# lucastrefezza/quadruplet-sentence-transformer

Measured on AMD Instinct MI355X. Metric: quadruplets/sec (seq_len=128, all-MiniLM-L6-v2) training step, higher is better.
Workload: dtype bf16; 1 GPU; all-MiniLM-L6-v2 dims (random-init), 64 quadruplets/GPU x 1 GPU, seq_len=128, fwd + gamma-quadruplet loss + bwd + clip + AdamW, dropout 0.1 on hidden states and attention probabilities as the reference's train() mode (BASELINE.json configs[1]); global_batch=64, seq_len=128, parallelism=dp1, precision=bf16 MFMA operands, fp32 accumulate/residual/LN/softmax/loss/optimizer, launch=eager

## Files before the change

### include/qst_kernels.h

```cpp
#pragma once
#include <stddef.h>
#include <stdint.h>

#ifdef __cplusplus
extern "C" {
#endif

enum {
    QST_EPI_BF16 = 0,
    QST_EPI_F32_RESID = 1,
    QST_EPI_GELU = 2,
    QST_EPI_GELU_BWD = 3,
    QST_EPI_F32_RESID_BF16 = 4,
    QST_EPI_GELU_MX = 5,
    QST_EPI_GELU_MX_TRAIN = 6
};

typedef struct {
    const uint32_t* state;
    uint32_t site;
    uint32_t thr16;
} QstDrop;
#define QST_DROP_SITE_EMBED 0xE0u
#define QST_DROP_SITE_ATTN_OUT(layer) (4u * (uint32_t)(layer) + 0u)
// ... 19 lines not shown
    void* C3;
    void* C4;
    const void* B2;
    int32_t b2_n0;
    int32_t sat16;
} QstGemmArgs;

int qst_gemm_nt(const QstGemmArgs* a, int epi, void* stream);
int qst_gemm_nt_f8(const QstGemmArgs* a, int epi, void* stream);
int qst_quant_mx(const void* src, int src_is_bf16, int64_t rows, int K, void* q, void* scales, void* stream);
typedef struct {
    const float* gamma;
    const float* beta;
    float eps;
    void* xhat;
    float* rstd;
    float* partials;
} QstLnEpi;
int qst_gemm_nt_ln_supported(int N);
int qst_gemm_nt_ln_block_rows(int N);
int qst_gemm_nt_ln_block_rows_m(int N, int M);
int qst_gemm_nt_ln(const QstGemmArgs* a, const QstLnEpi* ln, int mode, void* stream);
int qst_gemm_nt8_ln_supported(int N);
int qst_gemm_nt8_ln_block_rows(int M, int N);
int qst_gemm_nt8_ln(const QstGemmArgs* a, const QstLnEpi* ln, int mode, void* stream);
int qst_gemm_nt8_ln_timeouts(void);
int qst_gemm_nt8_f8_ln(const QstGemmArgs* a, const QstLnEpi* ln, void* stream);
typedef struct {
    const void* A;
    const void* B1;
    const void* B2;
    const float* bias1;
    const float* bias2;
    const float* resid;
    const void* aux;
    void* save_gp;
    void* save_h;
    float* C;
    void* C2;
    int32_t M, H, I;
    int32_t diag;
} QstFfnArgs;
int qst_ffn_chain_supported(int H, int I);
int qst_ffn_chain(const QstFfnArgs* a, const QstLnEpi* ln, int mode, void* stream);
int qst_gemm_tn(const QstGemmArgs* a, void* stream);
#define QST_TN_MAX_PROB 8
typedef struct {
    int32_t nprob;
    int32_t splits;
    int32_t total_tiles;
    int32_t ranges_per_xcd;
    int32_t tiles[QST_TN_MAX_PROB];
    QstGemmArgs prob[QST_TN_MAX_PROB];
} QstTnGroup;
int qst_gemm_tn_group(const QstTnGroup* grp, void* stream);

int qst_gemm8_stagger(int cycles);
int qst_gemm8_ln_store(int mode);
int qst_gemm_nt8_supported(const QstGemmArgs* a, int epi);
int qst_gemm_nt8(const QstGemmArgs* a, int epi, int tile, void* stream);
int qst_gemm_tn8_group(const QstTnGroup* grp, void* stream);
int qst_gemm_nt8_f8(const QstGemmArgs* a, int epi, int tile, void* stream);
int qst_gemm8_mode(int mode);

int qst_embed_ln_fwd(const int64_t* ids, const int64_t* type_ids, const int32_t* pos_ids,
                     const float* word_emb, const float* pos_emb, const float* type_emb,
                     const float* gamma, const float* beta, float eps, int M, int H,
                     float* y, void* y_bf16, void* xhat_bf16, float* rstd, void* stream);
int qst_embed_ln_fwd_drop(const int64_t* ids, const int64_t* type_ids, const int32_t* pos_ids,
                          const float* word_emb, const float* pos_emb, const float* type_emb,
                          const float* gamma, const float* beta, float eps, int M, int H,
                          float* y, void* y_bf16, void* xhat_bf16, float* rstd, const QstDrop* drop, void* stream);
int qst_ln_fwd(const float* s, const float* gamma, const float* beta, float eps, int M, int H,
               float* y, void* y_bf16, void* xhat_bf16, float* rstd, void* stream);
int qst_ln_fwd_mx(const float* s, const float* gamma, const float* beta, float eps, int M, int H,
                  float* y, void* y_bf16, void* yq, void* ys, void* stream);
int qst_embed_ln_fwd_mx(const int64_t* ids, const int64_t* type_ids, const int32_t* pos_ids,
                        const float* word_emb, const float* pos_emb, const float* type_emb,
                        const float* gamma, const float* beta, float eps, int M, int H,
                        float* y, void* y_bf16, void* yq, void* ys, void* stream);
int qst_ln_fwd_mx_train(const float* s, const float* gamma, const float* beta, float eps, int M, int H, float* y,
                        void* y_bf16, void* xhat_bf16, float* rstd, void* yq, void* ys, void* stream);
int qst_embed_ln_fwd_mx_train(const int64_t* ids, const int64_t* type_ids, const int32_t* pos_ids,
                              const float* word_emb, const float* pos_emb, const float* type_emb,
                              const float* gamma, const float* beta, float eps, int M, int H, float* y,
                              void* y_bf16, void* xhat_bf16, float* rstd, void* yq, void* ys,
                              const QstDrop* drop , void* stream);
size_t qst_ln_bwd_scratch_bytes(int M, int H);
int qst_ln_bwd(const float* dy, const void* xhat_bf16, const float* rstd, const float* gamma, int M, int H,
               float* ds, void* ds_bf16, float* dgamma, float* dbeta, float* scratch, void* stream);
int qst_ln_bwd_drop(const float* dy, const void* xhat_bf16, const float* rstd, const float* gamma, int M, int H,
                    float* ds, void* ds_bf16, float* dgamma, float* dbeta, float* scratch,
                    const QstDrop* drop_in, const QstDrop* drop_out, void* stream);
#define QST_LN_BATCH_MAX 32
typedef struct {
    int32_t count, H, nblocks;
    const float* partials[QST_LN_BATCH_MAX];
    float* dgamma[QST_LN_BATCH_MAX];
    float* dbeta[QST_LN_BATCH_MAX];
    int32_t nblocks_each[QST_LN_BATCH_MAX];
} QstLnReduceBatch;
int qst_ln_bwd_reduce_batch(const QstLnReduceBatch* b, void* stream);
int qst_embed_bwd(const float* ds, const int64_t* ids, const int64_t* type_ids, const int32_t* pos_ids,
                  int nseq, int L, int H, int num_types, float* dword, float* dpos, float* dtype_, void* stream);
int qst_position_ids(const int64_t* ids, int nseq, int L, int arch, int pad_id, int32_t* pos_ids, void* stream);
int qst_forward_prologue(const int64_t* ids, int nseq, int L, int arch, int pad_id, int32_t* pos_ids,
                         uint32_t* drop_state, uint32_t* drop_snapshot, void* stream);

// ... 121 lines not shown
```

### quadruplet-sentence-transformer_amd/_lib.py

```python
from __future__ import annotations

import ctypes as C
import os
from typing import Optional

_HERE = os.path.dirname(os.path.abspath(__file__))
LIB_PATH = os.path.join(_HERE, "libqst.so")

c_i64p = C.POINTER(C.c_int64)
c_i32p = C.POINTER(C.c_int32)
c_f32p = C.POINTER(C.c_float)
vp = C.c_void_p


class QstError(RuntimeError):
    pass


class QstConfig(C.Structure):
    _fields_ = [("arch", C.c_int32), ("vocab_size", C.c_int32), ("hidden_size", C.c_int32),
                ("num_layers", C.c_int32), ("num_heads", C.c_int32), ("intermediate_size", C.c_int32),
                ("max_position", C.c_int32), ("type_vocab_size", C.c_int32), ("layer_norm_eps", C.c_float),
                ("normalize", C.c_int32), ("rel_buckets", C.c_int32), ("rel_max_distance", C.c_int32),
                ("pad_token_id", C.c_int32), ("precision", C.c_int32)]


class QstDrop(C.Structure):
    _fields_ = [("state", vp), ("site", C.c_uint32), ("thr16", C.c_uint32)]


class QstAttnDesc(C.Structure):
    _fields_ = [("qkv", vp), ("mask", vp), ("rel_pos", vp), ("nseq", C.c_int32), ("L", C.c_int32), ("A", C.c_int32),
                ("d", C.c_int32), ("ctx", vp), ("lse", vp), ("dctx", vp), ("dqkv", vp), ("drel", vp), ("delta_scratch", vp),
                ("force_split", C.c_int32), ("drop", QstDrop)]


class QstGemmArgs(C.Structure):
    _fields_ = [("A", vp), ("B", vp), ("C", vp), ("C2", vp), ("aux", vp), ("bias", vp), ("resid", vp),
                ("colsum", vp), ("M", C.c_int32), ("N", C.c_int32), ("K", C.c_int32), ("lda", C.c_int32),
                ("ldb", C.c_int32), ("ldc", C.c_int32), ("ldr", C.c_int32), ("splits", C.c_int32), ("bscale", vp),
                ("drop", QstDrop), ("drop_where", C.c_int32), ("C3", vp), ("C4", vp), ("B2", vp), ("b2_n0", C.c_int32), ("sat16", C.c_int32)]


class QstLnEpi(C.Structure):
    _fields_ = [("gamma", vp), ("beta", vp), ("eps", C.c_float), ("xhat", vp), ("rstd", vp), ("partials", vp)]


class QstFfnArgs(C.Structure):
    _fields_ = [("A", vp), ("B1", vp), ("B2", vp), ("bias1", vp), ("bias2", vp), ("resid", vp), ("aux", vp),
                ("save_gp", vp), ("save_h", vp), ("C", vp), ("C2", vp), ("M", C.c_int32), ("H", C.c_int32), ("I", C.c_int32),
                ("diag", C.c_int32)]


class QstLnReduceBatch(C.Structure):
    _fields_ = [("count", C.c_int32), ("H", C.c_int32), ("nblocks", C.c_int32), ("partials", vp * 32), ("dgamma", vp * 32),
                ("dbeta", vp * 32), ("nblocks_each", C.c_int32 * 32)]


class QstTnGroup(C.Structure):
    _fields_ = [("nprob", C.c_int32), ("splits", C.c_int32), ("total_tiles", C.c_int32), ("ranges_per_xcd", C.c_int32),
                ("tiles", C.c_int32 * 8),
                ("prob", QstGemmArgs * 8)]


SIGNATURES = {
    "qst_strerror": (C.c_char_p, [C.c_int]),
    "qst_last_hip_error": (C.c_int, []),
    "qst_version": (C.c_int, []),
    "qst_arena_elems": (C.c_int64, [C.POINTER(QstConfig)]),
    "qst_arena_num_segments": (C.c_int, [C.POINTER(QstConfig)]),
    "qst_arena_segment": (C.c_int, [C.POINTER(QstConfig), C.c_int, C.POINTER(C.c_char_p), c_i64p, c_i64p, c_i32p, c_i32p]),
    "qst_shadow_elems": (C.c_int64, [C.POINTER(QstConfig)]),
    "qst_encoder_create": (C.c_int, [C.POINTER(QstConfig), C.POINTER(vp)]),
    "qst_encoder_destroy": (None, [vp]),
    "qst_encoder_saved_bytes": (C.c_size_t, [vp, C.c_int, C.c_int, C.c_int]),
    "qst_encoder_bwd_workspace_bytes": (C.c_size_t, [vp, C.c_int, C.c_int]),
    "qst_refresh_shadow": (C.c_int, [vp, vp, vp, vp]),
    "qst_refresh_shadow_mx": (C.c_int, [vp, vp, vp, vp]),
    "qst_encoder_forward": (C.c_int, [vp, vp, vp, vp, C.c_int, C.c_int, vp, vp, vp, vp, vp, C.c_size_t, C.c_int, vp]),
    "qst_encoder_backward": (C.c_int, [vp, vp, vp, vp, C.c_int, C.c_int, vp, vp, vp, vp, vp, C.c_size_t, vp, C.c_size_t, vp]),
    "qst_encoder_backward_partial": (C.c_int, [vp, vp, vp, vp, C.c_int, C.c_int, vp, vp, vp, vp, vp, C.c_size_t, vp, C.c_size_t,
                                               C.c_int, C.c_int, C.c_int, C.c_int, vp]),
    "qst_encoder_backward_stage": (C.c_int, [vp, vp, vp, vp, C.c_int, C.c_int, vp, vp, vp, vp, vp, C.c_size_t, vp, C.c_size_t,
                                             C.c_int, C.c_int, C.c_int, vp]),
    "qst_quadruplet_loss": (C.c_int, [vp, vp, vp, vp, C.c_int, C.c_int, C.c_float, C.c_float, C.c_float, C.c_float,
                                      C.c_float, C.c_int, C.c_int, vp, vp, vp, vp, vp, vp, vp, vp]),
    "qst_pair_metric": (C.c_int, [vp, vp, C.c_int, C.c_int, C.c_int, vp, vp, vp, vp, vp]),
    "qst_pair_loss": (C.c_int, [vp, vp, vp, C.c_int, C.c_int, C.c_int, C.c_int, C.c_float, C.c_int, vp, vp, vp, vp, vp, vp]),
    "qst_triplet_loss": (C.c_int, [vp, vp, vp, C.c_int, C.c_int, C.c_int, C.c_float, C.c_int, vp, vp, vp, vp, vp, vp, vp]),
    "qst_quadruplet_eval": (C.c_int, [vp, vp, vp, vp, C.c_int, C.c_int, vp, vp, vp, vp]),
    "qst_mnrl_workspace_bytes": (C.c_size_t, [C.c_int, C.c_int, C.c_int]),
    "qst_mnrl_loss": (C.c_int, [vp, vp, C.c_int, C.c_int, C.c_int, C.c_int, C.c_float, C.c_int, vp, vp, vp, vp, vp, C.c_size_t,
                                vp]),
    "qst_batch_triplet_workspace_bytes": (C.c_size_t, [C.c_int, C.c_int]),
    "qst_batch_triplet_loss": (C.c_int, [vp, vp, C.c_int, C.c_int, C.c_int, C.c_int, C.c_float, vp, vp, vp, vp, vp, C.c_size_t,
                                         vp]),
    "qst_embed_mse": (C.c_int, [vp, vp, C.c_int, C.c_int, vp, vp, vp, vp, vp]),
    "qst_margin_mse_loss": (C.c_int, [vp, vp, vp, vp, C.c_int, C.c_int, C.c_int, C.c_int, vp, vp, vp, vp, vp, vp, vp, vp]),
    "qst_clip_adamw_step": (C.c_int, [vp, vp, vp, vp, vp, C.c_float, C.c_float, C.c_float, C.c_float, C.c_float,
                                      C.c_float, C.c_float, C.c_int64, vp, vp, vp]),
    "qst_shadow8_bytes": (C.c_int64, [C.POINTER(QstConfig)]),
    "qst_clip_adamw_step_sched": (C.c_int, [vp, vp, vp, vp, vp, C.c_float, C.c_float, C.c_float, C.c_float, C.c_float,
                                            C.c_float, C.c_float, C.c_int64, C.c_int64, vp, vp, vp, vp]),
    "qst_topk_workspace_bytes": (C.c_size_t, [C.c_int, C.c_int, C.c_int]),
    "qst_topk_scores": (C.c_int, [vp, vp, C.c_int, C.c_int, C.c_int, C.c_int, C.c_int, vp, vp, vp, C.c_size_t, vp]),
    "qst_topk_scores_capped": (C.c_int, [vp, vp, C.c_int, C.c_int, C.c_int, C.c_int, C.c_int, C.c_float, vp, vp, vp,
                                         C.c_size_t, vp]),
    "qst_score_workspace_bytes": (C.c_size_t, [C.c_int, C.c_int, C.c_int]),
    "qst_score_matrix": (C.c_int, [vp, vp, C.c_int, C.c_int, C.c_int, C.c_int, vp, C.c_int64, vp, C.c_size_t, vp]),
    "qst_gemm_nt": (C.c_int, [C.POINTER(QstGemmArgs), C.c_int, vp]),
    "qst_gemm_nt_f8": (C.c_int, [C.POINTER(QstGemmArgs), C.c_int, vp]),
    "qst_quant_mx": (C.c_int, [vp, C.c_int, C.c_int64, C.c_int, vp, vp, vp]),
    "qst_gemm_nt_ln_supported": (C.c_int, [C.c_int]),
    "qst_gemm_nt_ln": (C.c_int, [C.POINTER(QstGemmArgs), C.POINTER(QstLnEpi), C.c_int, vp]),
    "qst_gemm_nt_ln_block_rows": (C.c_int, [C.c_int]),
    "qst_gemm_nt_ln_block_rows_m": (C.c_int, [C.c_int, C.c_int]),
    "qst_gemm_nt8_ln_block_rows": (C.c_int, [C.c_int, C.c_int]),
    "qst_gemm8_stagger": (C.c_int, [C.c_int]),
    "qst_gemm8_ln_store": (C.c_int, [C.c_int]),
    "qst_gemm_nt8_ln_supported": (C.c_int, [C.c_int]),
    "qst_gemm_nt8_ln": (C.c_int, [C.POINTER(QstGemmArgs), C.POINTER(QstLnEpi), C.c_int, vp]),
    "qst_gemm_nt8_ln_timeouts": (C.c_int, []),
    "qst_gemm_nt8_f8_ln": (C.c_int, [C.POINTER(QstGemmArgs), C.POINTER(QstLnEpi), vp]),
    "qst_ffn_chain_supported": (C.c_int, [C.c_int, C.c_int]),
    "qst_ffn_chain": (C.c_int, [C.POINTER(QstFfnArgs), C.POINTER(QstLnEpi), C.c_int, vp]),
    "qst_gemm_tn": (C.c_int, [C.POINTER(QstGemmArgs), vp]),
    "qst_gemm_tn_group": (C.c_int, [C.POINTER(QstTnGroup), vp]),
    "qst_gemm_nt8_supported": (C.c_int, [C.POINTER(QstGemmArgs), C.c_int]),
    "qst_gemm_nt8": (C.c_int, [C.POINTER(QstGemmArgs), C.c_int, C.c_int, vp]),
    "qst_gemm_tn8_group": (C.c_int, [C.POINTER(QstTnGroup), vp]),
    "qst_gemm_nt8_f8": (C.c_int, [C.POINTER(QstGemmArgs), C.c_int, C.c_int, vp]),
    "qst_gemm8_mode": (C.c_int, [C.c_int]),
    "qst_embed_ln_fwd": (C.c_int, [vp, vp, vp, vp, vp, vp, vp, vp, C.c_float, C.c_int, C.c_int, vp, vp, vp, vp, vp]),
    "qst_embed_ln_fwd_drop": (C.c_int, [vp, vp, vp, vp, vp, vp, vp, vp, C.c_float, C.c_int, C.c_int, vp, vp, vp, vp,
                                        C.POINTER(QstDrop), vp]),
    "qst_ln_fwd_mx": (C.c_int, [vp, vp, vp, C.c_float, C.c_int, C.c_int, vp, vp, vp, vp, vp]),
    "qst_embed_ln_fwd_mx": (C.c_int, [vp, vp, vp, vp, vp, vp, vp, vp, C.c_float, C.c_int, C.c_int, vp, vp, vp, vp, vp]),
    "qst_ln_fwd_mx_train": (C.c_int, [vp, vp, vp, C.c_float, C.c_int, C.c_int, vp, vp, vp, vp, vp, vp, vp]),
    "qst_embed_ln_fwd_mx_train": (C.c_int, [vp, vp, vp, vp, vp, vp, vp, vp, C.c_float, C.c_int, C.c_int, vp, vp, vp, vp, vp, vp,
                                            vp, vp]),
    "qst_ln_fwd": (C.c_int, [vp, vp, vp, C.c_float, C.c_int, C.c_int, vp, vp, vp, vp, vp]),
    "qst_ln_bwd_scratch_bytes": (C.c_size_t, [C.c_int, C.c_int]),
    "qst_ln_bwd_reduce_batch": (C.c_int, [vp, vp]),
    "qst_ln_bwd": (C.c_int, [vp, vp, vp, vp, C.c_int, C.c_int, vp, vp, vp, vp, vp, vp]),
    "qst_ln_bwd_drop": (C.c_int, [vp, vp, vp, vp, C.c_int, C.c_int, vp, vp, vp, vp, vp, C.POINTER(QstDrop), C.POINTER(QstDrop), vp]),
    "qst_embed_bwd": (C.c_int, [vp, vp, vp, vp, C.c_int, C.c_int, C.c_int, C.c_int, vp, vp, vp, vp]),
    "qst_position_ids": (C.c_int, [vp, C.c_int, C.c_int, C.c_int, C.c_int, vp, vp]),
    "qst_forward_prologue": (C.c_int, [vp, C.c_int, C.c_int, C.c_int, C.c_int, vp, vp, vp, vp]),
    "qst_pool_norm_fwd": (C.c_int, [vp, vp, C.c_int, C.c_int, C.c_int, C.c_int, vp, vp, vp]),
    "qst_pool_norm_bwd": (C.c_int, [vp, vp, vp, C.c_int, C.c_int, C.c_int, C.c_int, vp, vp]),
    "qst_pool_fwd": (C.c_int, [vp, vp, C.c_int, C.c_int, C.c_int, C.c_int, C.c_int, vp, vp, vp, vp]),
    "qst_pool_bwd": (C.c_int, [vp, vp, vp, vp, C.c_int, C.c_int, C.c_int, C.c_int, C.c_int, vp, vp]),
    "qst_attention_fwd": (C.c_int, [vp, vp, vp, C.c_int, C.c_int, C.c_int, C.c_int, vp, vp, vp]),
    "qst_attention_bwd": (C.c_int, [vp, vp, vp, vp, vp, vp, C.c_int, C.c_int, C.c_int, C.c_int, vp, vp, vp, vp]),
    "qst_attention_fwd_ex": (C.c_int, [C.POINTER(QstAttnDesc), vp]),
    "qst_attention_bwd_ex": (C.c_int, [C.POINTER(QstAttnDesc), vp]),
    "qst_dropout_multipliers": (C.c_int, [C.POINTER(QstDrop), C.c_int, C.c_int64, vp, vp]),
    "qst_abi_sizeof": (C.c_int64, [C.c_int]),
    "qst_normalize_rows": (C.c_int, [vp, C.c_int, C.c_int, vp, vp]),
    "qst_cls_head_fwd": (C.c_int, [vp, C.c_int64, C.c_int, C.c_int, vp, vp, vp, vp, C.c_int, C.c_int, C.c_int, vp, vp]),
    "qst_dropout_init": (C.c_int, [vp, C.c_uint64, vp]),
    "qst_dropout_advance": (C.c_int, [vp, vp]),
    "qst_encoder_set_dropout": (C.c_int, [vp, C.c_float, C.c_float, vp]),
    "qst_encoder_set_ffn_chain": (C.c_int, [vp, C.c_int]),
    "qst_encoder_set_ln_fusion": (C.c_int, [vp, C.c_int]),
    "qst_encoder_set_pooling": (C.c_int, [vp, C.c_int]),
    "qst_encoder_embedding_dim": (C.c_int, [vp]),
    "qst_transpose_f32": (C.c_int, [vp, C.c_int, C.c_int, C.c_int, vp, C.c_int, vp]),
    "qst_gelu_f32": (C.c_int, [vp, C.c_int64, vp, vp]),
    "qst_gelu_bwd_f32": (C.c_int, [vp, vp, C.c_int64, vp, vp]),
    "qst_colsum_f32": (C.c_int, [vp, C.c_int, C.c_int, C.c_int, vp, vp]),
    "qst_embed_sum_f32": (C.c_int, [vp, vp, vp, vp, vp, vp, C.c_int, C.c_int, vp, vp]),
    "qst_ln_bwd_f32": (C.c_int, [vp, vp, vp, C.c_float, C.c_int, C.c_int, vp, vp, vp, vp]),
    "qst_attention_bwd_f32": (C.c_int, [vp, vp, vp, vp, vp, C.c_int, C.c_int, C.c_int, C.c_int, vp, vp, vp]),
    "qst_attention_bwd_f32_drop": (C.c_int, [vp, vp, vp, vp, vp, C.c_int, C.c_int, C.c_int, C.c_int, vp, vp, vp, vp]),
    "qst_attention_bwd_x3_scratch_bytes": (C.c_size_t, [C.c_int, C.c_int, C.c_int]),
    "qst_attention_bwd_x3": (C.c_int, [vp, vp, vp, vp, vp, C.c_int, C.c_int, C.c_int, C.c_int, vp, vp, vp, vp, vp]),
    "qst_dropout_apply_f32": (C.c_int, [vp, vp, vp, C.c_int64, vp, vp]),
    "qst_comm_unique_id": (C.c_int, [vp]),
    "qst_comm_init": (C.c_int, [C.c_int, C.c_int, vp, C.POINTER(vp)]),
# ... 82 lines not shown
```

### quadruplet-sentence-transformer_amd/csrc/gemm.hip

```cpp
#include "qst_common.h"
#include "qst_kernels.h"

namespace {

constexpr uint32_t kOOB = 0x7FFFFFF0u;

typedef __attribute__((address_space(3))) void lds_void;
typedef __attribute__((ext_vector_type(2))) float f32x2;

template <bool ONCE = false>
__device__ __forceinline__ void dma16(__amdgpu_buffer_rsrc_t r, char* lds_wave_base, uint32_t voff, uint32_t soff) {
    __builtin_amdgcn_raw_ptr_buffer_load_lds(r, (lds_void*)lds_wave_base, 16, (int)voff, (int)soff, 0,
                                             (ONCE && QST_STREAM_LOADS) ? 2 : 0);
}
template <int N> __device__ __forceinline__ void wait_vmcnt() {
    if (N == 0) asm volatile("s_waitcnt vmcnt(0)" ::: "memory");
    else if (N == 4) asm volatile("s_waitcnt vmcnt(4)" ::: "memory");
    else asm volatile("s_waitcnt vmcnt(8)" ::: "memory");
}
template <int N> __device__ __forceinline__ void wait_vmcnt_n() {
    if (N == 0) asm volatile("s_waitcnt vmcnt(0)" ::: "memory");
    else if (N == 6) asm volatile("s_waitcnt vmcnt(6)" ::: "memory");
    else if (N == 12) asm volatile("s_waitcnt vmcnt(12)" ::: "memory");
    else if (N == 18) asm volatile("s_waitcnt vmcnt(18)" ::: "memory");
    else asm volatile("s_waitcnt vmcnt(24)" ::: "memory");
}
__device__ __forceinline__ void wait_stage(int stages_behind) {
    if (stages_behind >= 2) wait_vmcnt<8>();
    else if (stages_behind == 1) wait_vmcnt<4>();
    else wait_vmcnt<0>();
}

__device__ __forceinline__ int xcd_remap(int b, int nwg) {
    const int q = nwg >> 3, r = nwg & 7, x = b & 7;
    return (x < r ? x * (q + 1) : r * (q + 1) + (x - r) * q) + (b >> 3);
}

constexpr int NBK = 64;
constexpr int NT_STG_LD = 100;
__device__ __forceinline__ uint32_t nt_off(int row, int chunk) {
    return (uint32_t)(row * 128 + ((chunk ^ ((row >> 1) & 7)) << 4));
}

struct NoHook { __device__ __forceinline__ void operator()() const {} };
template <int WAVES_M, int WAVES_N, typename HOOK = NoHook, bool A_ONCE = false, int A_SLOTS = 2, bool SPLITW = true>
__device__ __forceinline__ void nt_mainloop(const QstGemmArgs& g, char* smem, int m0, int n0, f32x16 (&acc)[2][3],
                                            HOOK after_first_issue = HOOK()) {
    constexpr int NBM = 64 * WAVES_M, NBN = 96 * WAVES_N, NW = WAVES_M * WAVES_N;
    constexpr int NT_A_BYTES = NBM * NBK * 2, NT_B_BYTES = NBN * NBK * 2;
    constexpr int NT_STAGE = NT_A_BYTES + NT_B_BYTES;
    constexpr int A_PER_WAVE = (NBM / 8) / NW;
    constexpr int B_PER_WAVE = (NBN / 8) / NW;
// ... 724 lines not shown
                    s2 += v[t][0] * x[t][0] + v[t][1] * x[t][1];
                }
                const float m1 = wave_sum(s1) * inv_n, m2 = wave_sum(s2) * inv_n;
                if (m < g.M) {
#pragma unroll
                    for (int t = 0; t < 3; ++t) {
                        const int c = 2 * (lane + 64 * t);
                        f32x2 o;
                        o[0] = rs[i][k] * (v[t][0] - m1 - x[t][0] * m2);
                        o[1] = rs[i][k] * (v[t][1] - m1 - x[t][1] * m2);
                        st_stream((f32x2*)((float*)g.C + (size_t)m * g.ldc + c), o);
                        if (g.C2) {
                            if (DROP && dwhere == 2) {
                                float k0, k1;
                                drop_pair(dc, (uint32_t)m * LN_N + c, k0, k1);
                                o[0] *= k0; o[1] *= k1;
                            }
                            st_stream((uint32_t*)((op16*)g.C2 + (size_t)m * g.ldc + c), pack_op2(o[0], o[1]));
                        }
                    }
                }
            }
        }
        LN_STAMP(4 + 2 * i);
    }
    LN_STAMP(7);
    if (MODE == 1 && e.partials) {
        __syncthreads();
        float* red = (float*)smem;
#pragma unroll
        for (int t = 0; t < 3; ++t) {
            *(f32x2*)(red + (wave * 2 + 0) * LN_N + 2 * (lane + 64 * t)) = ag[t];
            *(f32x2*)(red + (wave * 2 + 1) * LN_N + 2 * (lane + 64 * t)) = ab[t];
        }
        __syncthreads();
        for (int c = tid; c < 2 * LN_N; c += 512) {
            const int which = c / LN_N, n = c - which * LN_N;
            float a = 0.f;
#pragma unroll
            for (int w = 0; w < 8; ++w) a += red[(w * 2 + which) * LN_N + n];
            e.partials[(size_t)blockIdx.x * 2 * LN_N + c] = a;
        }
    }
}

constexpr int TT = 192, TBK = 64, TSTAGES = 3;
constexpr int TT_TILE = TBK * TT * 2;
constexpr int TT_STAGE = 2 * TT_TILE;
constexpr int TT_LDS = TSTAGES * TT_STAGE;
__device__ __forceinline__ int tn_swz(int row) { return ((row >> 1) & 1) << 2; }
__device__ __forceinline__ uint32_t tn_off(int row, int chunk) {
    return (uint32_t)(row * 384 + ((chunk ^ tn_swz(row)) << 4));
}
__device__ __forceinline__ op16x4 lds_tr16(const char* p) {
    return lds_tr16_op(p);
}
__device__ __forceinline__ op16x4 lds_tr16_at(uint32_t a) {
    typedef __attribute__((ext_vector_type(4))) __bf16 raw4;
    return __builtin_bit_cast(op16x4, __builtin_amdgcn_ds_read_tr16_b64_v4bf16((__attribute__((address_space(3))) raw4*)(uintptr_t)a));
}

__global__ __launch_bounds__(512, 1) void gemm_tn_group_kernel(QstTnGroup grp) {
    extern __shared__ __attribute__((aligned(16))) char smem[];
    const int tid = threadIdx.x, lane = tid & 63;
    const int wave = __builtin_amdgcn_readfirstlane(tid >> 6);
    const int wm = (wave >> 1) & 1, wn = wave & 1;
    const int xcd = blockIdx.x & 7, jloc = blockIdx.x >> 3;
    const int wg_per_range = (int)(gridDim.x >> 3) / grp.ranges_per_xcd;
    const int range = xcd + 8 * (jloc / wg_per_range);
    const int jr = jloc % wg_per_range;
    const int M = grp.prob[0].M;
    const int per = (((M + grp.splits - 1) / grp.splits) + TBK - 1) / TBK * TBK;
    const int mbeg = range * per, mend = min(M, mbeg + per);
    if (mbeg >= mend) return;
    const int S = (mend - mbeg + TBK - 1) / TBK;
    const int W = wg_per_range, T = grp.total_tiles;
    const int a_full = T / W, b_left = T % W;
    const int pieces = b_left > 0 ? max(1, W / b_left) : 1;
    const int ntasks = a_full + ((b_left > 0 && jr / pieces < b_left) ? 1 : 0);

    const int li = lane & 15, q = li >> 2, p = li & 3, gsel = (lane >> 4) & 1, fh = lane >> 5;
    const int fr = lane & 31;

#pragma unroll 1
    for (int task = 0; task < ntasks; ++task) {
        int tile, s0, s1;
        if (task < a_full) { tile = task * W + jr; s0 = 0; s1 = S; }
        else {
            tile = a_full * W + jr / pieces;
            const int pc = jr % pieces;
            const int per_piece = (S + pieces - 1) / pieces;
            s0 = pc * per_piece; s1 = min(S, s0 + per_piece);
        }
        const int nm = s1 - s0;
        if (nm <= 0) continue;
        int pi = 0;
#pragma unroll 1
        while (pi + 1 < grp.nprob && tile >= grp.tiles[pi]) { tile -= grp.tiles[pi]; ++pi; }
        const QstGemmArgs& g = grp.prob[pi];
        const int ntk = (g.K + TT - 1) / TT;
        const int n0 = (tile / ntk) * TT, k0 = (tile % ntk) * TT;
        const int row0 = mbeg + s0 * TBK;

        if (wave >= 4) {
            const bool isA = wave < 6;
            const int half = wave & 1;
            const int ld = isA ? g.lda : g.ldb, c0 = isA ? n0 : k0, width = isA ? g.N : g.K;
            const op16* base = (const op16*)(isA ? g.A : g.B) + (size_t)row0 * ld + c0;
            const uint32_t bytes = (uint32_t)min((size_t)(mend - row0) * ld * 2u - (size_t)c0 * 2u, (size_t)0x7FFFFF00u);
            const __amdgpu_buffer_rsrc_t rs = make_rsrc(base, bytes);
            constexpr int NDMA = TBK * 24 / 64 / 2;
            uint32_t vo[NDMA];
#pragma unroll
            for (int b = 0; b < 3; ++b) {
                const int pp = (half * NDMA + b) * 64 + lane;
                const int row = pp / 24, chunk = (pp % 24) ^ tn_swz(row);
                const bool ok = c0 + chunk * 8 < width;
#pragma unroll
                for (int t = b; t < NDMA; t += 3)
                    vo[t] = ok ? (uint32_t)(row + 8 * (t / 3)) * ld * 2u + chunk * 16u : kOOB;
            }
            auto issue = [&](int mt) {
                char* st = smem + (mt % TSTAGES) * TT_STAGE + (isA ? 0 : TT_TILE);
                const uint32_t so = (uint32_t)mt * TBK * ld * 2u;
#pragma unroll
                for (int t = 0; t < NDMA; ++t) dma16(rs, st + (half * NDMA + t) * 1024, vo[t], so);
            };
            constexpr int AHEAD = TSTAGES - 1;
#pragma unroll 1
            for (int st = 0; st < AHEAD && st < nm; ++st) issue(st);
#pragma unroll 1
            for (int mt = 0; mt < nm; ++mt) {
                const int younger = min(AHEAD - 1, nm - 1 - mt);
                if (younger >= 1) wait_vmcnt_n<12>(); else wait_vmcnt_n<0>();
                __builtin_amdgcn_s_barrier();
                if (mt + AHEAD < nm) issue(mt + AHEAD);
            }
            __builtin_amdgcn_s_barrier();
            continue;
        }

        f32x16 acc[3][3];
        float bsum[3] = {0.f, 0.f, 0.f};
#pragma unroll
        for (int i = 0; i < 3; ++i)
#pragma unroll
            for (int j = 0; j < 3; ++j)
#pragma unroll
                for (int r = 0; r < 16; ++r) acc[i][j][r] = 0.f;
        const bool do_bias = (g.colsum != nullptr) && (k0 == 0) && (wn == 0);
        uint32_t la[3], lb[3];
        {
            const uint32_t lr = (uint32_t)(8 * fh + q) * 384u + 8u * (p & 1), g2 = gsel * 2 + (p >> 1);
#pragma unroll
            for (int i = 0; i < 3; ++i) {
                la[i] = lr + (uint32_t)(((wm * 12 + i * 4 + g2) ^ tn_swz(q)) << 4);
                lb[i] = lr + TT_TILE + (uint32_t)(((wn * 12 + i * 4 + g2) ^ tn_swz(q)) << 4);
            }
        }
        uint32_t slot = (uint32_t)(uintptr_t)(__attribute__((address_space(3))) char*)smem;

        for (int mt = 0; mt < nm; ++mt) {
            __builtin_amdgcn_s_barrier();
            uint32_t ra[3], rb[3];
#pragma unroll
            for (int i = 0; i < 3; ++i) {
                ra[i] = slot + la[i]; rb[i] = slot + lb[i];
                asm volatile("" : "+v"(ra[i]), "+v"(rb[i]));
            }
            slot = (mt % TSTAGES == TSTAGES - 1) ? slot - (TSTAGES - 1) * TT_STAGE : slot + TT_STAGE;
            op16x8 fa[2][3], fb[2][3];
#define TN_LOAD(ks_, set_)                                                                                  \
    do {                                                                                                    \
        _Pragma("unroll") for (int i = 0; i < 3; ++i) {                                                     \
            _Pragma("unroll") for (int jj = 0; jj < 2; ++jj) {                                              \
                const op16x4 ta = lds_tr16_at(ra[i] + ((ks_) * 16 + 4 * jj) * 384);                         \
                const op16x4 tb = lds_tr16_at(rb[i] + ((ks_) * 16 + 4 * jj) * 384);                         \
                _Pragma("unroll") for (int e = 0; e < 4; ++e) { fa[set_][i][jj * 4 + e] = ta[e]; fb[set_][i][jj * 4 + e] = tb[e]; } \
            }                                                                                               \
        }                                                                                                   \
    } while (0)
#define TN_MFMA(set_)                                                                                       \
    do {                                                                                                    \
        _Pragma("unroll") for (int i = 0; i < 3; ++i)                                                       \
            _Pragma("unroll") for (int j = 0; j < 3; ++j)                                                   \
                acc[i][j] = mfma32_op(fa[set_][i], fb[set_][j], acc[i][j]); \
        if (do_bias) {    \
            _Pragma("unroll") for (int i = 0; i < 3; ++i)                                                   \
                _Pragma("unroll") for (int e = 0; e < 8; ++e) bsum[i] += (float)fa[set_][i][e];             \
        }                                                                                                   \
    } while (0)
            TN_LOAD(0, 0);
            TN_LOAD(1, 1);
            TN_MFMA(0);
            TN_LOAD(2, 0);
            TN_MFMA(1);
            TN_LOAD(3, 1);
            TN_MFMA(0);
            TN_MFMA(1);
#undef TN_LOAD
#undef TN_MFMA
            if (!do_bias) {
                __builtin_amdgcn_sched_group_barrier(0x100, 12, 0);
#pragma unroll
                for (int rep = 0; rep < 3; ++rep) {
#pragma unroll
                    for (int u = 0; u < 3; ++u) {
                        __builtin_amdgcn_sched_group_barrier(0x008, 1, 0);
                        __builtin_amdgcn_sched_group_barrier(0x100, 2, 0);
                    }
#pragma unroll
                    for (int u = 0; u < 6; ++u) {
                        __builtin_amdgcn_sched_group_barrier(0x008, 1, 0);
                        __builtin_amdgcn_sched_group_barrier(0x100, 1, 0);
                    }
                }
                __builtin_amdgcn_sched_group_barrier(0x008, 9, 0);
            }
        }
        __builtin_amdgcn_s_barrier();

        float* C = (float*)g.C;
#pragma unroll
        for (int j = 0; j < 3; ++j) {
            const int k = k0 + wn * 96 + j * 32 + fr;
            if (k >= g.K) continue;
#pragma unroll
            for (int i = 0; i < 3; ++i) {
#pragma unroll
                for (int r = 0; r < 16; ++r) {
                    const int n = n0 + wm * 96 + i * 32 + (r & 3) + 8 * (r >> 2) + 4 * fh;
                    if (n < g.N) atomicAdd(&C[(size_t)n * g.ldc + k], acc[i][j][r]);
                }
            }
        }
        if (do_bias) {
#pragma unroll
            for (int i = 0; i < 3; ++i) {
                const float t = bsum[i] + swap32(bsum[i]);
                const int n = n0 + wm * 96 + i * 32 + fr;
                if (fh == 0 && n < g.N) atomicAdd(&g.colsum[n], t);
            }
        }
    }
}

}

int qst_gemm8_mode_get();
static bool nt8_auto(const QstGemmArgs* a, int epi) {
    const int64_t tiles = (int64_t)((a->M + 255) / 256) * ((a->N + 255) / 256);
    if (tiles < 1024 || a->K < 768) return false;
    if (epi == QST_EPI_BF16) return true;
    if (epi == QST_EPI_GELU) return a->N >= 2304;
    if (epi == QST_EPI_GELU_BWD) return a->N >= 2304 && tiles >= 4096;
    if (epi == QST_EPI_F32_RESID || epi == QST_EPI_F32_RESID_BF16) return a->K >= 2304;
    return false;
}

template <int EPI, int WAVES_M, int WAVES_N = 2, int TI = 2>
static int launch_nt(const QstGemmArgs* a, hipStream_t st) {
    constexpr int NBM = 32 * TI * WAVES_M, NBN = 96 * WAVES_N;
    constexpr int lds = 2 * (NBM + NBN) * (TI == 4 ? 32 : NBK) * 2;
    static QstLdsAttr attr;
    if (int rc = qst_ensure_lds(attr, (const void*)gemm_nt_kernel<EPI, WAVES_M, WAVES_N, TI>, lds)) return rc;
    const int ntm = (a->M + NBM - 1) / NBM, ntn = (a->N + NBN - 1) / NBN;
    gemm_nt_kernel<EPI, WAVES_M, WAVES_N, TI><<<dim3(ntm * ntn), dim3(64 * WAVES_M * WAVES_N), lds, st>>>(*a);
    QST_LAUNCH_CHECK();
    return QST_OK;
}

extern "C" int QST_K(qst_gemm_nt)(const QstGemmArgs* a, int epi, void* stream) {
// ... 88 lines not shown
}

extern "C" int qst_quant_mx(const void* src, int src_is_bf16, int64_t rows, int K, void* q, void* scales, void* stream) {
    if (!src || !q || !scales || rows <= 0 || K <= 0) return QST_ERR_BAD_ARG;
    if (K % 32 != 0) return QST_ERR_UNSUPPORTED;
    const int64_t n8 = rows * K / 8;
    const unsigned grid = (unsigned)((n8 + 255) / 256);
    if (src_is_bf16) quant_mx_kernel<op16><<<grid, 256, 0, (hipStream_t)stream>>>((const op16*)src, n8, rows, K, (uint8_t*)q, (uint8_t*)scales);
    else quant_mx_kernel<float><<<grid, 256, 0, (hipStream_t)stream>>>((const float*)src, n8, rows, K, (uint8_t*)q, (uint8_t*)scales);
    QST_LAUNCH_CHECK();
    return QST_OK;
}

extern "C" int qst_gemm_nt_ln_supported(int N) { return (N == LN_N || qst_gemm_nt8_ln_supported(N)) ? 1 : 0; }
extern "C" int qst_gemm_nt_ln_block_rows(int N) { return N == LN_N ? 128 : 256; }
extern "C" int qst_gemm_nt_ln_block_rows_m(int N, int M) { return N == LN_N ? 128 : qst_gemm_nt8_ln_block_rows(M, N); }
#endif

extern "C" int QST_K(qst_gemm_nt_ln)(const QstGemmArgs* a, const QstLnEpi* ln, int mode, void* stream) {
    if (!a || !ln || !a->A || !a->B || !a->C || !ln->gamma || a->M <= 0 || a->K <= 0) return QST_ERR_BAD_ARG;
    if (mode != 0 && mode != 1) return QST_ERR_BAD_ARG;
    if (mode == 0 && !ln->beta) return QST_ERR_BAD_ARG;
    if (mode == 1 && (!ln->xhat || !ln->rstd)) return QST_ERR_BAD_ARG;
    if (a->N != LN_N && qst_gemm_nt8_ln_supported(a->N)) return QST_K(qst_gemm_nt8_ln)(a, ln, mode, stream);
    if (a->N != LN_N || a->K % NBK != 0 || a->lda % 8 != 0 || a->ldb % 8 != 0 || a->ldc % 2 != 0 || (a->resid && a->ldr % 2 != 0))
        return QST_ERR_UNSUPPORTED;
    if ((int64_t)128 * a->lda * 2 >= 0x7FFFFF00LL || (int64_t)LN_N * a->ldb * 2 >= 0x7FFFFF00LL) return QST_ERR_UNSUPPORTED;
    if (a->drop.thr16 && a->drop.state) {
        if (a->drop.thr16 > 65535u || (int64_t)a->M * a->N >= ((int64_t)1 << 32)) return QST_ERR_UNSUPPORTED;
        if (mode == 0 ? a->drop_where != 1 : (a->drop_where != 2 && a->drop_where != 3)) return QST_ERR_BAD_ARG;
    }
    static QstLdsAttr attr0, attr1, attr01, attr12, attr13;
    const int ntm = (a->M + 127) / 128;
    if (a->drop.thr16 && a->drop.state) {
        if (int rc = qst_ensure_lds(attr01, (const void*)gemm_nt_ln_kernel<0, 1>, LN_LDS)) return rc;
        if (int rc = qst_ensure_lds(attr12, (const void*)gemm_nt_ln_kernel<1, 2>, LN_LDS)) return rc;
        if (int rc = qst_ensure_lds(attr13, (const void*)gemm_nt_ln_kernel<1, 3>, LN_LDS)) return rc;
        if (mode == 0) gemm_nt_ln_kernel<0, 1><<<dim3(ntm), dim3(512), LN_LDS, (hipStream_t)stream>>>(*a, *ln);
        else if (a->drop_where == 2) gemm_nt_ln_kernel<1, 2><<<dim3(ntm), dim3(512), LN_LDS, (hipStream_t)stream>>>(*a, *ln);
        else gemm_nt_ln_kernel<1, 3><<<dim3(ntm), dim3(512), LN_LDS, (hipStream_t)stream>>>(*a, *ln);
        QST_LAUNCH_CHECK();
        return QST_OK;
    }
    if (int rc = qst_ensure_lds(attr0, (const void*)gemm_nt_ln_kernel<0>, LN_LDS)) return rc;
    if (int rc = qst_ensure_lds(attr1, (const void*)gemm_nt_ln_kernel<1>, LN_LDS)) return rc;
    if (mode == 0) gemm_nt_ln_kernel<0><<<dim3(ntm), dim3(512), LN_LDS, (hipStream_t)stream>>>(*a, *ln);
    else gemm_nt_ln_kernel<1><<<dim3(ntm), dim3(512), LN_LDS, (hipStream_t)stream>>>(*a, *ln);
    QST_LAUNCH_CHECK();
    return QST_OK;
}

static bool tn8_auto(const QstTnGroup* g) { (void)g; return false; }

extern "C" int QST_K(qst_gemm_tn_group)(const QstTnGroup* grp_in, void* stream) {
    if (!grp_in || grp_in->nprob <= 0 || grp_in->nprob > QST_TN_MAX_PROB) return QST_ERR_BAD_ARG;
    {
        const int mode = qst_gemm8_mode_get();
        if (mode >= 0 ? (mode & 2) != 0 : tn8_auto(grp_in)) return QST_K(qst_gemm_tn8_group)(grp_in, stream);
    }
    QstTnGroup g = *grp_in;
    g.total_tiles = 0;
    for (int i = 0; i < g.nprob; ++i) {
        const QstGemmArgs& a = g.prob[i];
        if (!a.A || !a.B || !a.C || a.M <= 0 || a.N <= 0 || a.K <= 0 || a.M != g.prob[0].M) return QST_ERR_BAD_ARG;
        if (a.lda % 8 != 0 || a.ldb % 8 != 0 || a.N % 8 != 0 || a.K % 8 != 0) return QST_ERR_UNSUPPORTED;
        if ((int64_t)a.M * a.lda * 2 >= 0x7FFFFF00LL || (int64_t)a.M * a.ldb * 2 >= 0x7FFFFF00LL) return QST_ERR_UNSUPPORTED;
        g.tiles[i] = ((a.N + TT - 1) / TT) * ((a.K + TT - 1) / TT);
        g.total_tiles += g.tiles[i];
    }
    const int M = g.prob[0].M;
    if (g.splits <= 0) {
        g.splits = 8;
    }
    g.splits = (g.splits + 7) / 8 * 8;
    g.ranges_per_xcd = g.splits / 8;
    const int64_t stages = ((int64_t)(M + g.splits - 1) / g.splits + TBK - 1) / TBK;
    int64_t wg_per_range = 32 / g.ranges_per_xcd;
    if (wg_per_range < 1) wg_per_range = 1;
    const int64_t work = (int64_t)g.total_tiles * stages;
    if (wg_per_range > work) wg_per_range = work < 1 ? 1 : work;
    const int grid = (int)(8 * g.ranges_per_xcd * wg_per_range);
    static QstLdsAttr attr;
    if (int rc = qst_ensure_lds(attr, (const void*)gemm_tn_group_kernel, TT_LDS)) return rc;
    gemm_tn_group_kernel<<<dim3(grid), dim3(512), TT_LDS, (hipStream_t)stream>>>(g);
    QST_LAUNCH_CHECK();
    return QST_OK;
}

extern "C" int QST_K(qst_gemm_tn)(const QstGemmArgs* a, void* stream) {
    if (!a) return QST_ERR_BAD_ARG;
    QstTnGroup g{};
    g.nprob = 1;
    g.splits = a->splits;
    g.prob[0] = *a;
    return QST_K(qst_gemm_tn_group)(&g, stream);
}
```

Before: 14330 quadruplets/s.

## Skew split-K row ranges and reorder leftover tiles in grouped TN GEMM

Replaces the uniform per-range row split in the weight-gradient TN GEMM with a skewed stage partition, so per-XCD ranges get unequal row counts. It also adds a by-piece ordering for leftover tiles, where odd pieces run their leftover task first, to balance workgroup finish times. The bias column-sum is now split across both wn halves by k-step parity and uses bf16 dot2 instead of scalar adds, which lets the MFMA schedule barriers stay on for bias tiles. The added template specialisation raises code size, and the skew changes how the atomic-add contention is distributed.

```diff
diff --git a/include/qst_kernels.h b/include/qst_kernels.h
--- a/include/qst_kernels.h
+++ b/include/qst_kernels.h
@@ -95,8 +95,11 @@
     int32_t ranges_per_xcd;
     int32_t tiles[QST_TN_MAX_PROB];
     QstGemmArgs prob[QST_TN_MAX_PROB];
+    int32_t skew;
+    int32_t order;
 } QstTnGroup;
 int qst_gemm_tn_group(const QstTnGroup* grp, void* stream);
+int qst_tn_group_ranges(const QstTnGroup* grp, int32_t* row_begin);
 
 int qst_gemm8_stagger(int cycles);
 int qst_gemm8_ln_store(int mode);
diff --git a/quadruplet-sentence-transformer_amd/_lib.py b/quadruplet-sentence-transformer_amd/_lib.py
--- a/quadruplet-sentence-transformer_amd/_lib.py
+++ b/quadruplet-sentence-transformer_amd/_lib.py
@@ -60,7 +60,8 @@
 class QstTnGroup(C.Structure):
     _fields_ = [("nprob", C.c_int32), ("splits", C.c_int32), ("total_tiles", C.c_int32), ("ranges_per_xcd", C.c_int32),
                 ("tiles", C.c_int32 * 8),
-                ("prob", QstGemmArgs * 8)]
+                ("prob", QstGemmArgs * 8),
+                ("skew", C.c_int32), ("order", C.c_int32)]
 
 
 SIGNATURES = {
@@ -126,6 +127,7 @@
     "qst_ffn_chain": (C.c_int, [C.POINTER(QstFfnArgs), C.POINTER(QstLnEpi), C.c_int, vp]),
     "qst_gemm_tn": (C.c_int, [C.POINTER(QstGemmArgs), vp]),
     "qst_gemm_tn_group": (C.c_int, [C.POINTER(QstTnGroup), vp]),
+    "qst_tn_group_ranges": (C.c_int, [C.POINTER(QstTnGroup), c_i32p]),
     "qst_gemm_nt8_supported": (C.c_int, [C.POINTER(QstGemmArgs), C.c_int]),
     "qst_gemm_nt8": (C.c_int, [C.POINTER(QstGemmArgs), C.c_int, C.c_int, vp]),
     "qst_gemm_tn8_group": (C.c_int, [C.POINTER(QstTnGroup), vp]),
diff --git a/quadruplet-sentence-transformer_amd/csrc/gemm.hip b/quadruplet-sentence-transformer_amd/csrc/gemm.hip
--- a/quadruplet-sentence-transformer_amd/csrc/gemm.hip
+++ b/quadruplet-sentence-transformer_amd/csrc/gemm.hip
@@ -1,3 +1,4 @@
+#include <type_traits>
 #include "qst_common.h"
 #include "qst_kernels.h"
 
@@ -828,12 +829,34 @@
 __device__ __forceinline__ uint32_t tn_off(int row, int chunk) {
     return (uint32_t)(row * 384 + ((chunk ^ tn_swz(row)) << 4));
 }
+__device__ __forceinline__ float add_pair(op16 a, op16 b, float c) {
+    const op16x2 v = {a, b}, one = {(op16)1.0f, (op16)1.0f};
+#if QST_OP_F16
+    return __builtin_amdgcn_fdot2(v, one, c, false);
+#else
+    return __builtin_amdgcn_fdot2_f32_bf16(v, one, c, false);
+#endif
+}
 __device__ __forceinline__ op16x4 lds_tr16(const char* p) {
     return lds_tr16_op(p);
 }
 __device__ __forceinline__ op16x4 lds_tr16_at(uint32_t a) {
     typedef __attribute__((ext_vector_type(4))) __bf16 raw4;
     return __builtin_bit_cast(op16x4, __builtin_amdgcn_ds_read_tr16_b64_v4bf16((__attribute__((address_space(3))) raw4*)(uintptr_t)a));
+}
+
+__host__ __device__ inline int tn_range_stage(int stages, int splits, int skew, int r) {
+    const int base = stages / splits, extra = stages % splits;
+    int s = r * base + (r > splits - extra ? r - (splits - extra) : 0);
+    if (skew > 0 && splits == 8) {
+        const int m = r < 8 - r ? r : 8 - r;
+        s -= skew * (m * (9 - m) / 2);
+    }
+    return s;
+}
+__host__ __device__ inline int tn_skew_max(int stages, int splits) {
+    const int base = stages / splits;
+    return splits == 8 && base > 1 ? (base - 1) / 4 : 0;
 }
 
 __global__ __launch_bounds__(512, 1) void gemm_tn_group_kernel(QstTnGroup grp) {
@@ -846,14 +869,19 @@
     const int range = xcd + 8 * (jloc / wg_per_range);
     const int jr = jloc % wg_per_range;
     const int M = grp.prob[0].M;
-    const int per = (((M + grp.splits - 1) / grp.splits) + TBK - 1) / TBK * TBK;
-    const int mbeg = range * per, mend = min(M, mbeg + per);
+    const int stages_m = (M + TBK - 1) / TBK;
+    const int mbeg = min(M, TBK * tn_range_stage(stages_m, grp.splits, grp.skew, range));
+    const int mend = min(M, TBK * tn_range_stage(stages_m, grp.splits, grp.skew, range + 1));
     if (mbeg >= mend) return;
     const int S = (mend - mbeg + TBK - 1) / TBK;
     const int W = wg_per_range, T = grp.total_tiles;
     const int a_full = T / W, b_left = T % W;
     const int pieces = b_left > 0 ? max(1, W / b_left) : 1;
-    const int ntasks = a_full + ((b_left > 0 && jr / pieces < b_left) ? 1 : 0);
+    const bool by_piece = grp.order == 2 && b_left > 0;
+    const int lt = by_piece ? jr % b_left : jr / pieces, lp = by_piece ? jr / b_left : jr % pieces;
+    const bool has_left = b_left > 0 && (by_piece ? lp < pieces : lt < b_left);
+    const bool left_first = by_piece && has_left && (lp & 1);
+    const int ntasks = a_full + (has_left ? 1 : 0);
 
     const int li = lane & 15, q = li >> 2, p = li & 3, gsel = (lane >> 4) & 1, fh = lane >> 5;
     const int fr = lane & 31;
@@ -861,12 +889,12 @@
 #pragma unroll 1
     for (int task = 0; task < ntasks; ++task) {
         int tile, s0, s1;
-        if (task < a_full) { tile = task * W + jr; s0 = 0; s1 = S; }
+        const int wt = left_first ? (task == 0 ? a_full : task - 1) : task;
+        if (wt < a_full) { tile = wt * W + jr; s0 = 0; s1 = S; }
         else {
-            tile = a_full * W + jr / pieces;
-            const int pc = jr % pieces;
+            tile = a_full * W + lt;
             const int per_piece = (S + pieces - 1) / pieces;
-            s0 = pc * per_piece; s1 = min(S, s0 + per_piece);
+            s0 = lp * per_piece; s1 = min(S, s0 + per_piece);
         }
         const int nm = s1 - s0;
         if (nm <= 0) continue;
@@ -924,7 +952,7 @@
             for (int j = 0; j < 3; ++j)
 #pragma unroll
                 for (int r = 0; r < 16; ++r) acc[i][j][r] = 0.f;
-        const bool do_bias = (g.colsum != nullptr) && (k0 == 0) && (wn == 0);
+        const bool do_bias = (g.colsum != nullptr) && (k0 == 0);
         uint32_t la[3], lb[3];
         {
             const uint32_t lr = (uint32_t)(8 * fh + q) * 384u + 8u * (p & 1), g2 = gsel * 2 + (p >> 1);
@@ -936,6 +964,8 @@
         }
         uint32_t slot = (uint32_t)(uintptr_t)(__attribute__((address_space(3))) char*)smem;
 
+        auto run_stages = [&](auto bias_tag) __attribute__((always_inline)) {
+        constexpr int BIAS = decltype(bias_tag)::value;
         for (int mt = 0; mt < nm; ++mt) {
             __builtin_amdgcn_s_barrier();
             uint32_t ra[3], rb[3];
@@ -956,44 +986,46 @@
             }                                                                                               \
         }                                                                                                   \
     } while (0)
-#define TN_MFMA(set_)                                                                                       \
+#define TN_MFMA(ks_, set_)                                                                                    \
     do {                                                                                                    \
         _Pragma("unroll") for (int i = 0; i < 3; ++i)                                                       \
             _Pragma("unroll") for (int j = 0; j < 3; ++j)                                                   \
                 acc[i][j] = mfma32_op(fa[set_][i], fb[set_][j], acc[i][j]); \
-        if (do_bias) {    \
+        if (BIAS == 1 + ((ks_) & 1)) {    \
             _Pragma("unroll") for (int i = 0; i < 3; ++i)                                                   \
-                _Pragma("unroll") for (int e = 0; e < 8; ++e) bsum[i] += (float)fa[set_][i][e];             \
+                _Pragma("unroll") for (int e = 0; e < 8; e += 2) bsum[i] = add_pair(fa[set_][i][e], fa[set_][i][e + 1], bsum[i]); \
         }                                                                                                   \
     } while (0)
             TN_LOAD(0, 0);
             TN_LOAD(1, 1);
-            TN_MFMA(0);
+            TN_MFMA(0, 0);
             TN_LOAD(2, 0);
-            TN_MFMA(1);
+            TN_MFMA(1, 1);
             TN_LOAD(3, 1);
-            TN_MFMA(0);
-            TN_MFMA(1);
+            TN_MFMA(2, 0);
+            TN_MFMA(3, 1);
 #undef TN_LOAD
 #undef TN_MFMA
-            if (!do_bias) {
-                __builtin_amdgcn_sched_group_barrier(0x100, 12, 0);
-#pragma unroll
-                for (int rep = 0; rep < 3; ++rep) {
-#pragma unroll
-                    for (int u = 0; u < 3; ++u) {
-                        __builtin_amdgcn_sched_group_barrier(0x008, 1, 0);
-                        __builtin_amdgcn_sched_group_barrier(0x100, 2, 0);
-                    }
-#pragma unroll
-                    for (int u = 0; u < 6; ++u) {
-                        __builtin_amdgcn_sched_group_barrier(0x008, 1, 0);
-                        __builtin_amdgcn_sched_group_barrier(0x100, 1, 0);
-                    }
-                }
-                __builtin_amdgcn_sched_group_barrier(0x008, 9, 0);
-            }
-        }
+            __builtin_amdgcn_sched_group_barrier(0x100, 12, 0);
+#pragma unroll
+            for (int rep = 0; rep < 3; ++rep) {
+#pragma unroll
+                for (int u = 0; u < 3; ++u) {
+                    __builtin_amdgcn_sched_group_barrier(0x008, 1, 0);
+                    __builtin_amdgcn_sched_group_barrier(0x100, 2, 0);
+                }
+#pragma unroll
+                for (int u = 0; u < 6; ++u) {
+                    __builtin_amdgcn_sched_group_barrier(0x008, 1, 0);
+                    __builtin_amdgcn_sched_group_barrier(0x100, 1, 0);
+                }
+            }
+            __builtin_amdgcn_sched_group_barrier(0x008, 9, 0);
+        }
+        };
+        if (!do_bias) run_stages(std::integral_constant<int, 0>{});
+        else if (wn == 0) run_stages(std::integral_constant<int, 1>{});
+        else run_stages(std::integral_constant<int, 2>{});
         __builtin_amdgcn_s_barrier();
 
         float* C = (float*)g.C;
@@ -1188,6 +1220,41 @@
 
 static bool tn8_auto(const QstTnGroup* g) { (void)g; return false; }
 
+static int tn_auto_skew(int total_tiles, int base) { return base < 16 || total_tiles < 32 ? 0 : total_tiles < 64 ? 2 : 1; }
+static int tn_auto_order(int total_tiles, int base) { return base < 16 || total_tiles < 32 ? 1 : 2; }
+
+static int tn_plan(QstTnGroup* g, bool launch) {
+    if (g->nprob <= 0 || g->nprob > QST_TN_MAX_PROB) return QST_ERR_BAD_ARG;
+    g->total_tiles = 0;
+    for (int i = 0; i < g->nprob; ++i) {
+        const QstGemmArgs& a = g->prob[i];
+        if ((launch && (!a.A || !a.B || !a.C)) || a.M <= 0 || a.N <= 0 || a.K <= 0 || a.M != g->prob[0].M) return QST_ERR_BAD_ARG;
+        if ((launch && (a.lda % 8 != 0 || a.ldb % 8 != 0)) || a.N % 8 != 0 || a.K % 8 != 0) return QST_ERR_UNSUPPORTED;
+        if (launch && ((int64_t)a.M * a.lda * 2 >= 0x7FFFFF00LL || (int64_t)a.M * a.ldb * 2 >= 0x7FFFFF00LL)) return QST_ERR_UNSUPPORTED;
+        g->tiles[i] = ((a.N + TT - 1) / TT) * ((a.K + TT - 1) / TT);
+        g->total_tiles += g->tiles[i];
+    }
+    if (g->splits <= 0) g->splits = 8;
+    g->splits = (g->splits + 7) / 8 * 8;
+    g->ranges_per_xcd = g->splits / 8;
+    const int stages_m = (g->prob[0].M + TBK - 1) / TBK, base = stages_m / g->splits;
+    if (g->skew == 0) g->skew = tn_auto_skew(g->total_tiles, base);
+    g->skew = g->skew < 0 ? 0 : std::min(g->skew, tn_skew_max(stages_m, g->splits));
+    if (g->order != 1 && g->order != 2) g->order = tn_auto_order(g->total_tiles, base);
+    return QST_OK;
+}
+
+#if !QST_OP_F16
+extern "C" int qst_tn_group_ranges(const QstTnGroup* grp_in, int32_t* row_begin) {
+    if (!grp_in || !row_begin) return QST_ERR_BAD_ARG;
+    QstTnGroup g = *grp_in;
+    if (int rc = tn_plan(&g, false)) return rc;
+    const int M = g.prob[0].M, stages_m = (M + TBK - 1) / TBK;
+    for (int r = 0; r <= g.splits; ++r) row_begin[r] = std::min(M, TBK * tn_range_stage(stages_m, g.splits, g.skew, r));
+    return g.skew;
+}
+#endif
+
 extern "C" int QST_K(qst_gemm_tn_group)(const QstTnGroup* grp_in, void* stream) {
     if (!grp_in || grp_in->nprob <= 0 || grp_in->nprob > QST_TN_MAX_PROB) return QST_ERR_BAD_ARG;
     {
@@ -1195,22 +1262,10 @@
         if (mode >= 0 ? (mode & 2) != 0 : tn8_auto(grp_in)) return QST_K(qst_gemm_tn8_group)(grp_in, stream);
     }
     QstTnGroup g = *grp_in;
-    g.total_tiles = 0;
-    for (int i = 0; i < g.nprob; ++i) {
-        const QstGemmArgs& a = g.prob[i];
-        if (!a.A || !a.B || !a.C || a.M <= 0 || a.N <= 0 || a.K <= 0 || a.M != g.prob[0].M) return QST_ERR_BAD_ARG;
-        if (a.lda % 8 != 0 || a.ldb % 8 != 0 || a.N % 8 != 0 || a.K % 8 != 0) return QST_ERR_UNSUPPORTED;
-        if ((int64_t)a.M * a.lda * 2 >= 0x7FFFFF00LL || (int64_t)a.M * a.ldb * 2 >= 0x7FFFFF00LL) return QST_ERR_UNSUPPORTED;
-        g.tiles[i] = ((a.N + TT - 1) / TT) * ((a.K + TT - 1) / TT);
-        g.total_tiles += g.tiles[i];
-    }
+    if (int rc = tn_plan(&g, true)) return rc;
     const int M = g.prob[0].M;
-    if (g.splits <= 0) {
-        g.splits = 8;
-    }
-    g.splits = (g.splits + 7) / 8 * 8;
-    g.ranges_per_xcd = g.splits / 8;
-    const int64_t stages = ((int64_t)(M + g.splits - 1) / g.splits + TBK - 1) / TBK;
+    const int stages_m = (M + TBK - 1) / TBK;
+    const int64_t stages = tn_range_stage(stages_m, g.splits, g.skew, g.splits) - tn_range_stage(stages_m, g.splits, g.skew, g.splits - 1);
     int64_t wg_per_range = 32 / g.ranges_per_xcd;
     if (wg_per_range < 1) wg_per_range = 1;
     const int64_t work = (int64_t)g.total_tiles * stages;
```

After: 14640 quadruplets/s, median of 6. 1.02x the previous value.
